# NVlabs/FoundationPose

Measured on NVIDIA H100. Metric: pose-hypotheses/sec at 640x480 RGB-D, 252 hyp, 5 refine iters, higher is better.
Workload: dtype f16

## Files before the change

foundationpose_b200/csrc/fp_attn_tc.cu:

```cuda
#include "fp_attn.cuh"
#include "fp_common.cuh"
#include "fp_gemm.cuh"
#include "fp_wgmma.cuh"

namespace fp {

int encode_map_f16(CUtensorMap* map, const void* base, int rank, const uint64_t* dims, const uint64_t* strides_bytes,
                   const uint32_t* box);
int num_sms();

namespace {

constexpr int T = 400;
constexpr int DH = 128;
constexpr int kQTiles = (T + 127) / 128;
constexpr int kKeys = 80;
constexpr int kChunks = T / kKeys;
constexpr int kKVSlab = kKeys * 128;
constexpr int kKVStage = 4 * kKVSlab;
constexpr int kKVStages = 3;
constexpr int kQSlab = 128 * 128;
constexpr int kQStage = 2 * kQSlab;
constexpr int kQStages = 2;
constexpr int kOffKV = 0;
constexpr int kOffQ = kOffKV + kKVStages * kKVStage;
constexpr int kOffBar = kOffQ + kQStages * kQStage;
constexpr int kSmem = kOffBar + 256 + 1024;
constexpr int kThreadsTc = 384;

__device__ __forceinline__ void tma_load_3d(const CUtensorMap* map, uint64_t* bar, void* dst, int c0, int c1, int c2) {
  asm volatile(
      "cp.async.bulk.tensor.3d.shared::cluster.global.mbarrier::complete_tx::bytes [%0], [%1, {%3, %4, %5}], [%2];" ::"r"(
          smem_u32(dst)),
      "l"(reinterpret_cast<uint64_t>(map)), "r"(smem_u32(bar)), "r"(c0), "r"(c1), "r"(c2)
      : "memory");
}
__device__ __forceinline__ void tma_store_4d(const CUtensorMap* map, const void* src, int c0, int c1, int c2, int c3) {
  asm volatile("cp.async.bulk.tensor.4d.global.shared::cta.bulk_group [%0, {%2, %3, %4, %5}], [%1];" ::"l"(
                   reinterpret_cast<uint64_t>(map)),
               "r"(smem_u32(src)), "r"(c0), "r"(c1), "r"(c2), "r"(c3)
               : "memory");
}

struct TcParams {
  int q_col, k_col, v_col;
  int group_col_stride;
  float scale_log2e;
  int B, H, G;
};

__global__ void __launch_bounds__(kThreadsTc, 1)
    attn_tc_kernel(const __grid_constant__ CUtensorMap map_kv,
                   const __grid_constant__ CUtensorMap map_q,
                   const __grid_constant__ CUtensorMap map_o,
                   const TcParams p) {
  extern __shared__ uint8_t smem_raw[];
  uint8_t* smem = reinterpret_cast<uint8_t*>((reinterpret_cast<uintptr_t>(smem_raw) + 1023) & ~uintptr_t(1023));
  uint64_t* bars = reinterpret_cast<uint64_t*>(smem + kOffBar);
  uint64_t* q_full = bars;
  uint64_t* q_empty = bars + kQStages;
  uint64_t* kv_full = bars + 2 * kQStages;
  uint64_t* kv_empty = bars + 2 * kQStages + kKVStages;

  const int total = p.B * p.H * p.G * kQTiles;

  if (threadIdx.x == 0) {
    tma_prefetch_desc(&map_kv);
    tma_prefetch_desc(&map_q);
    tma_prefetch_desc(&map_o);
    for (int i = 0; i < kQStages; ++i) {
      mbar_init(&q_full[i], 1);
      mbar_init(&q_empty[i], 2);
    }
    for (int i = 0; i < kKVStages; ++i) {
      mbar_init(&kv_full[i], 1);
      mbar_init(&kv_empty[i], 256);
    }
    mbar_fence_init();
  }
  __syncthreads();
  pdl_trigger();
  pdl_wait();

  auto unit = [&](int u, int& b, int& h, int& g, int& gcol, int& qt) {
    qt = u % kQTiles;
    const int w = u / kQTiles;
    b = w % p.B;
    h = (w / p.B) % p.H;
    g = w / (p.B * p.H);
    gcol = g * p.group_col_stride + h * DH;
  };

  if (threadIdx.x < 128) {
    if (threadIdx.x == 0) {
      int qs = 0, qph = 0, ks = 0, kph = 0;
      for (int u = blockIdx.x; u < total; u += gridDim.x) {
        int b, h, g, gcol, qt;
        unit(u, b, h, g, gcol, qt);
        mbar_wait(&q_empty[qs], qph ^ 1);
        mbar_expect_tx(&q_full[qs], kQStage);
        for (int s = 0; s < 2; ++s)
          tma_load_3d(&map_q, &q_full[qs], smem + kOffQ + qs * kQStage + s * kQSlab, gcol + p.q_col + s * 64, qt * 128, b);
        if (++qs == kQStages) {
          qs = 0;
          qph ^= 1;
        }
        for (int c = 0; c < kChunks; ++c) {
          mbar_wait(&kv_empty[ks], kph ^ 1);
          mbar_expect_tx(&kv_full[ks], kKVStage);
          uint8_t* st = smem + kOffKV + ks * kKVStage;
          for (int s = 0; s < 2; ++s) {
            tma_load_3d(&map_kv, &kv_full[ks], st + s * kKVSlab, gcol + p.k_col + s * 64, c * kKeys, b);
            tma_load_3d(&map_kv, &kv_full[ks], st + (2 + s) * kKVSlab, gcol + p.v_col + s * 64, c * kKeys, b);
          }
          if (++ks == kKVStages) {
            ks = 0;
            kph ^= 1;
          }
        }
      }
    }
    return;
  }

  const int ct = threadIdx.x - 128;
  const int cw = ct >> 7;
  const int lane = threadIdx.x & 31;
  const int r0 = 64 * cw + 16 * ((ct >> 5) & 3) + (lane >> 2);
  const int cq = 2 * (lane & 3);
  const bool leader = ((ct & 127) == 0);
  const float c = p.scale_log2e;
  float s_acc[kKeys / 2], o[DH / 2];
#pragma unroll
  for (int i = 0; i < kKeys / 2; ++i) s_acc[i] = 0.f;
  int qs = 0, qph = 0, ks = 0, kph = 0;
  for (int u = blockIdx.x; u < total; u += gridDim.x) {
    int b, h, g, gcol, qt;
    unit(u, b, h, g, gcol, qt);
#pragma unroll
    for (int i = 0; i < DH / 2; ++i) o[i] = 0.f;
    float m[2] = {-INFINITY, -INFINITY}, l[2] = {0.f, 0.f};
    mbar_wait(&q_full[qs], qph);
    const uint32_t qbase = smem_u32(smem + kOffQ + qs * kQStage) + (uint32_t)cw * 8192u;
    for (int ch = 0; ch < kChunks; ++ch) {
      mbar_wait(&kv_full[ks], kph);
      const uint32_t kvbase = smem_u32(smem + kOffKV + ks * kKVStage);
      wgmma_fence();
#pragma unroll
      for (int kk = 0; kk < 8; ++kk) {
        const int s = kk >> 2, k = kk & 3;
        Wgmma<kKeys>::ss(s_acc, gmma_desc_sw128(qbase + s * kQSlab) + (uint64_t)(2 * k),
                         gmma_desc_sw128(kvbase + s * kKVSlab) + (uint64_t)(2 * k), kk > 0 ? 1u : 0u);
      }
      wgmma_commit();
      wgmma_wait<0>();
      fence_regs(s_acc);
      float mx[2] = {m[0], m[1]};
#pragma unroll
      for (int j = 0; j < kKeys / 8; ++j) {
        mx[0] = fmaxf(mx[0], fmaxf(s_acc[4 * j], s_acc[4 * j + 1]));
        mx[1] = fmaxf(mx[1], fmaxf(s_acc[4 * j + 2], s_acc[4 * j + 3]));
      }
      float mc[2], alpha[2];
#pragma unroll
      for (int hh = 0; hh < 2; ++hh) {
        mx[hh] = fmaxf(mx[hh], __shfl_xor_sync(0xffffffffu, mx[hh], 1));
        mx[hh] = fmaxf(mx[hh], __shfl_xor_sync(0xffffffffu, mx[hh], 2));
        alpha[hh] = exp2f((m[hh] - mx[hh]) * c);
        m[hh] = mx[hh];
        mc[hh] = mx[hh] * c;
        l[hh] *= alpha[hh];
      }
#pragma unroll
      for (int j = 0; j < DH / 8; ++j) {
        o[4 * j] *= alpha[0];
        o[4 * j + 1] *= alpha[0];
        o[4 * j + 2] *= alpha[1];
        o[4 * j + 3] *= alpha[1];
      }
      uint32_t pa[kKeys / 16][4];
#pragma unroll
      for (int j = 0; j < kKeys / 8; ++j) {
#pragma unroll
        for (int hh = 0; hh < 2; ++hh) {
          const float p0 = exp2f(fmaf(s_acc[4 * j + 2 * hh], c, -mc[hh]));
          const float p1 = exp2f(fmaf(s_acc[4 * j + 2 * hh + 1], c, -mc[hh]));
          l[hh] += p0 + p1;
          pa[j >> 1][(j & 1) * 2 + hh] = pack_half2(p0, p1);
        }
      }
      wgmma_fence();
#pragma unroll
      for (int kk = 0; kk < kKeys / 16; ++kk)
        Wgmma<DH>::rs_mn(o, pa[kk], gmma_desc_mn_sw128(kvbase + 2 * kKVSlab + kk * 16 * 128, kKVSlab), 1u);
      wgmma_commit();
      wgmma_wait<0>();
      fence_regs(o);
      mbar_arrive(&kv_empty[ks]);
      if (++ks == kKVStages) {
        ks = 0;
        kph ^= 1;
      }
    }
    float inv[2];
#pragma unroll
    for (int hh = 0; hh < 2; ++hh) {
      l[hh] += __shfl_xor_sync(0xffffffffu, l[hh], 1);
      l[hh] += __shfl_xor_sync(0xffffffffu, l[hh], 2);
      inv[hh] = 1.f / l[hh];
    }
    uint8_t* qst = smem + kOffQ + qs * kQStage;
#pragma unroll
    for (int j = 0; j < DH / 8; ++j) {
#pragma unroll
      for (int hh = 0; hh < 2; ++hh) {
        const int row = r0 + 8 * hh;
        *reinterpret_cast<uint32_t*>(qst + (j >> 3) * kQSlab + row * 128 + ((((uint32_t)j & 7u) ^ (uint32_t)(row & 7)) << 4) +
                                     cq * 2) = pack_half2(o[4 * j + 2 * hh] * inv[hh], o[4 * j + 2 * hh + 1] * inv[hh]);
      }
    }
    asm volatile("fence.proxy.async.shared::cta;" ::: "memory");
    asm volatile("bar.sync %0, 128;" ::"r"(1 + cw) : "memory");
    if (leader) {
      for (int s = 0; s < 2; ++s)
        tma_store_4d(&map_o, qst + s * kQSlab + cw * 8192, h * DH + s * 64, qt * 128 + 64 * cw, b, g);
      asm volatile("cp.async.bulk.commit_group;" ::: "memory");
      asm volatile("cp.async.bulk.wait_group.read 0;" ::: "memory");
      mbar_arrive(&q_empty[qs]);
    }
    if (++qs == kQStages) {
      qs = 0;
      qph ^= 1;
    }
  }
  if (leader) asm volatile("cp.async.bulk.wait_group 0;" ::: "memory");
}

}

int attn_tc_launch(const AttnParams& p, cudaStream_t stream) {
  FP_REQUIRE(p.T == T && p.n_heads == 4, "wgmma attention is specialised for T=400, 4 heads of 128");
  FP_REQUIRE(p.ld_out == 512, "wgmma attention writes [*, 512] rows");
  static std::atomic<unsigned long long> attr_mask{0};
  if (!device_bit_test(attr_mask)) {
    FP_CUDA_OK(cudaFuncSetAttribute(attn_tc_kernel, cudaFuncAttributeMaxDynamicSharedMemorySize, kSmem));
    device_bit_set(attr_mask);
  }
  if (p.B == 0) return 0;
  CUtensorMap mkv, mq, mo;
  const uint64_t E = 2;
  uint64_t d3[3] = {(uint64_t)p.ld, (uint64_t)T, (uint64_t)p.B};
  uint64_t s3[2] = {(uint64_t)p.ld * E, (uint64_t)p.ld * E * T};
  uint32_t bkv[3] = {64, (uint32_t)kKeys, 1}, bq[3] = {64, 128, 1};
  int rc = encode_map_f16(&mkv, p.qkv, 3, d3, s3, bkv);
  if (rc) return rc;
  rc = encode_map_f16(&mq, p.qkv, 3, d3, s3, bq);
  if (rc) return rc;
  uint64_t d4[4] = {512, (uint64_t)T, (uint64_t)p.B, (uint64_t)p.n_groups};
  uint64_t s4[3] = {512 * E, 512 * E * T, (uint64_t)p.out_group_stride * E};
  if (p.n_groups == 1) s4[2] = 512 * E * T * p.B;
  uint32_t bo[4] = {64, 64, 1, 1};
  rc = encode_map_f16(&mo, p.out, 4, d4, s4, bo);
  if (rc) return rc;
  TcParams tp;
  tp.q_col = p.q_off;
  tp.k_col = p.k_off;
  tp.v_col = p.v_off;
  tp.group_col_stride = p.group_col_stride;
  tp.scale_log2e = p.scale * 1.4426950408889634f;
  tp.B = p.B;
  tp.H = p.n_heads;
  tp.G = p.n_groups;
  const int total = p.B * p.n_heads * p.n_groups * kQTiles;
  const int sms = num_sms();
  FP_REQUIRE(sms > 0, "no CUDA device");
  dim3 grid(total < sms ? total : sms);
  FP_CUDA_OK(launch_pdl(attn_tc_kernel, grid, dim3(kThreadsTc), kSmem, stream, 1, mkv, mq, mo, tp));
  note_launches(1);
  FP_CUDA_OK(cudaGetLastError());
  return 0;
}

}
```

Before: 3859.

## Rework wgmma attention into 64-row query blocks with split K/V rings

Adds a new default attention kernel where each consumer warpgroup handles a 64-row query block, and a scheduler packs the seven blocks of each pair of (batch, head, group) units into items, including a shared tail item. This avoids the padding waste of 128-row tiles over T=400 (four tiles covering 512 rows). K and V now flow through separate 4-stage rings, and the S=QK^T of the next chunk is issued before the softmax of the current one, so wgmma overlaps with exp work. The old kernel stays available behind an environment variable. The cost is more complex ring bookkeeping and smaller per-warpgroup tiles, which may lower tensor-core efficiency per instruction.

```diff
diff --git a/foundationpose_b200/csrc/fp_attn_tc.cu b/foundationpose_b200/csrc/fp_attn_tc.cu
--- a/foundationpose_b200/csrc/fp_attn_tc.cu
+++ b/foundationpose_b200/csrc/fp_attn_tc.cu
@@ -13,10 +13,35 @@
 
 constexpr int T = 400;
 constexpr int DH = 128;
-constexpr int kQTiles = (T + 127) / 128;
 constexpr int kKeys = 80;
 constexpr int kChunks = T / kKeys;
 constexpr int kKVSlab = kKeys * 128;
+constexpr int kThreadsTc = 384;
+
+__device__ __forceinline__ void tma_load_3d(const CUtensorMap* map, uint64_t* bar, void* dst, int c0, int c1, int c2) {
+  asm volatile(
+      "cp.async.bulk.tensor.3d.shared::cluster.global.mbarrier::complete_tx::bytes [%0], [%1, {%3, %4, %5}], [%2];" ::"r"(
+          smem_u32(dst)),
+      "l"(reinterpret_cast<uint64_t>(map)), "r"(smem_u32(bar)), "r"(c0), "r"(c1), "r"(c2)
+      : "memory");
+}
+__device__ __forceinline__ void tma_store_4d(const CUtensorMap* map, const void* src, int c0, int c1, int c2, int c3) {
+  asm volatile("cp.async.bulk.tensor.4d.global.shared::cta.bulk_group [%0, {%2, %3, %4, %5}], [%1];" ::"l"(
+                   reinterpret_cast<uint64_t>(map)),
+               "r"(smem_u32(src)), "r"(c0), "r"(c1), "r"(c2), "r"(c3)
+               : "memory");
+}
+
+struct TcParams {
+  int q_col, k_col, v_col;
+  int group_col_stride;
+  float scale_log2e;
+  int B, H, G;
+};
+
+namespace legacy {
+
+constexpr int kQTiles = (T + 127) / 128;
 constexpr int kKVStage = 4 * kKVSlab;
 constexpr int kKVStages = 3;
 constexpr int kQSlab = 128 * 128;
@@ -26,34 +51,12 @@
 constexpr int kOffQ = kOffKV + kKVStages * kKVStage;
 constexpr int kOffBar = kOffQ + kQStages * kQStage;
 constexpr int kSmem = kOffBar + 256 + 1024;
-constexpr int kThreadsTc = 384;
-
-__device__ __forceinline__ void tma_load_3d(const CUtensorMap* map, uint64_t* bar, void* dst, int c0, int c1, int c2) {
-  asm volatile(
-      "cp.async.bulk.tensor.3d.shared::cluster.global.mbarrier::complete_tx::bytes [%0], [%1, {%3, %4, %5}], [%2];" ::"r"(
-          smem_u32(dst)),
-      "l"(reinterpret_cast<uint64_t>(map)), "r"(smem_u32(bar)), "r"(c0), "r"(c1), "r"(c2)
-      : "memory");
-}
-__device__ __forceinline__ void tma_store_4d(const CUtensorMap* map, const void* src, int c0, int c1, int c2, int c3) {
-  asm volatile("cp.async.bulk.tensor.4d.global.shared::cta.bulk_group [%0, {%2, %3, %4, %5}], [%1];" ::"l"(
-                   reinterpret_cast<uint64_t>(map)),
-               "r"(smem_u32(src)), "r"(c0), "r"(c1), "r"(c2), "r"(c3)
-               : "memory");
-}
-
-struct TcParams {
-  int q_col, k_col, v_col;
-  int group_col_stride;
-  float scale_log2e;
-  int B, H, G;
-};
 
 __global__ void __launch_bounds__(kThreadsTc, 1)
-    attn_tc_kernel(const __grid_constant__ CUtensorMap map_kv,
-                   const __grid_constant__ CUtensorMap map_q,
-                   const __grid_constant__ CUtensorMap map_o,
-                   const TcParams p) {
+    attn_tc_kernel_legacy(const __grid_constant__ CUtensorMap map_kv,
+                          const __grid_constant__ CUtensorMap map_q,
+                          const __grid_constant__ CUtensorMap map_o,
+                          const TcParams p) {
   extern __shared__ uint8_t smem_raw[];
   uint8_t* smem = reinterpret_cast<uint8_t*>((reinterpret_cast<uintptr_t>(smem_raw) + 1023) & ~uintptr_t(1023));
   uint64_t* bars = reinterpret_cast<uint64_t*>(smem + kOffBar);
@@ -238,20 +241,337 @@
 
 }
 
+constexpr int kBlockRows = 64;
+constexpr int kUnitItems = 7;
+constexpr int kRingStages = 4;
+constexpr int kRingStage = 2 * kKVSlab;
+constexpr int kBlkSlab = kBlockRows * 128;
+constexpr int kBlkBuf = 2 * kBlkSlab;
+constexpr int kOffK = 0;
+constexpr int kOffV = kOffK + kRingStages * kRingStage;
+constexpr int kOffQ = kOffV + kRingStages * kRingStage;
+constexpr int kOffO = kOffQ + 2 * kBlkBuf;
+constexpr int kOffBar = kOffO + 2 * kBlkBuf;
+constexpr int kSmem = kOffBar + 256 + 1024;
+constexpr int kProducerRegs = 40;
+constexpr int kConsumerRegs = 232;
+
+struct TcItem {
+  int unit[2], blk[2];
+  bool two;
+};
+
+__device__ __forceinline__ TcItem tc_item(int i, int units) {
+  const int r = i % kUnitItems;
+  const int u0 = 2 * (i / kUnitItems), u1 = u0 + 1;
+  TcItem it;
+  if (r < 3 || (r < 6 && u1 < units)) {
+    const int u = r < 3 ? u0 : u1;
+    const int pr = r < 3 ? r : r - 3;
+    it.unit[0] = it.unit[1] = u;
+    it.blk[0] = 2 * pr;
+    it.blk[1] = 2 * pr + 1;
+    it.two = false;
+  } else {
+    it.unit[0] = u0;
+    it.blk[0] = it.blk[1] = 6;
+    it.unit[1] = u1 < units ? u1 : -1;
+    it.two = u1 < units;
+  }
+  return it;
+}
+
+__host__ __device__ __forceinline__ int tc_items(int units) { return kUnitItems * (units / 2) + (units & 1 ? 4 : 0); }
+
+struct Ring {
+  int stage = 0, phase = 0, pos = 0;
+
+  __device__ __forceinline__ int take(uint64_t* full) {
+    const int s = stage;
+    mbar_wait(&full[s], phase);
+    if (++stage == kRingStages) {
+      stage = 0;
+      phase ^= 1;
+    }
+    ++pos;
+    return s;
+  }
+  __device__ __forceinline__ int take_at(int at, uint64_t* full, uint64_t* empty) {
+    while (pos < at) mbar_arrive(&empty[take(full)]);
+    return take(full);
+  }
+  __device__ __forceinline__ void finish(int n, uint64_t* full, uint64_t* empty) {
+    while (pos < n) mbar_arrive(&empty[take(full)]);
+    pos = 0;
+  }
+};
+
+__global__ void __launch_bounds__(kThreadsTc, 1)
+    attn_tc_kernel(const __grid_constant__ CUtensorMap map_kv,
+                   const __grid_constant__ CUtensorMap map_q,
+                   const __grid_constant__ CUtensorMap map_o,
+                   const TcParams p) {
+  extern __shared__ uint8_t smem_raw[];
+  uint8_t* smem = reinterpret_cast<uint8_t*>((reinterpret_cast<uintptr_t>(smem_raw) + 1023) & ~uintptr_t(1023));
+  uint64_t* bars = reinterpret_cast<uint64_t*>(smem + kOffBar);
+  uint64_t* k_full = bars;
+  uint64_t* k_empty = bars + kRingStages;
+  uint64_t* v_full = bars + 2 * kRingStages;
+  uint64_t* v_empty = bars + 3 * kRingStages;
+  uint64_t* q_full = bars + 4 * kRingStages;
+  uint64_t* q_empty = q_full + 2;
+
+  const int units = p.B * p.H * p.G;
+  const int total = tc_items(units);
+
+  if (threadIdx.x == 0) {
+    tma_prefetch_desc(&map_kv);
+    tma_prefetch_desc(&map_q);
+    tma_prefetch_desc(&map_o);
+    for (int i = 0; i < kRingStages; ++i) {
+      mbar_init(&k_full[i], 1);
+      mbar_init(&k_empty[i], 256);
+      mbar_init(&v_full[i], 1);
+      mbar_init(&v_empty[i], 256);
+    }
+    for (int w = 0; w < 2; ++w) {
+      mbar_init(&q_full[w], 1);
+      mbar_init(&q_empty[w], 128);
+    }
+    mbar_fence_init();
+  }
+  __syncthreads();
+  pdl_trigger();
+  pdl_wait();
+
+  auto unit_cols = [&](int u, int& b, int& h, int& g, int& gcol) {
+    b = u % p.B;
+    h = (u / p.B) % p.H;
+    g = u / (p.B * p.H);
+    gcol = g * p.group_col_stride + h * DH;
+  };
+
+  if (threadIdx.x < 128) {
+    regs_release<kProducerRegs>();
+    if (threadIdx.x == 0) {
+      int ks = 0, kph = 0, vs = 0, vph = 0;
+      uint32_t qph[2] = {0, 0};
+      auto fill = [&](uint64_t* full, uint64_t* empty, int& st, int& ph, int off, int col, int chunk, int b) {
+        mbar_wait(&empty[st], ph ^ 1);
+        mbar_expect_tx(&full[st], kRingStage);
+        for (int s = 0; s < 2; ++s)
+          tma_load_3d(&map_kv, &full[st], smem + off + st * kRingStage + s * kKVSlab, col + s * 64, chunk * kKeys, b);
+        if (++st == kRingStages) {
+          st = 0;
+          ph ^= 1;
+        }
+      };
+      for (int i = blockIdx.x; i < total; i += gridDim.x) {
+        const TcItem it = tc_item(i, units);
+        int b[2], gcol[2];
+#pragma unroll
+        for (int w = 0; w < 2; ++w) {
+          if (it.unit[w] < 0) continue;
+          int h, g;
+          unit_cols(it.unit[w], b[w], h, g, gcol[w]);
+          mbar_wait(&q_empty[w], qph[w] ^ 1);
+          qph[w] ^= 1;
+          mbar_expect_tx(&q_full[w], kBlkBuf);
+          for (int s = 0; s < 2; ++s)
+            tma_load_3d(&map_q, &q_full[w], smem + kOffQ + w * kBlkBuf + s * kBlkSlab, gcol[w] + p.q_col + s * 64,
+                        it.blk[w] * kBlockRows, b[w]);
+        }
+        const int streams = it.two ? 2 : 1;
+        for (int c = 0; c <= kChunks; ++c) {
+          if (c < kChunks)
+#pragma unroll
+            for (int w = 0; w < 2; ++w)
+              if (w < streams) fill(k_full, k_empty, ks, kph, kOffK, gcol[w] + p.k_col, c, b[w]);
+          if (c > 0)
+#pragma unroll
+            for (int w = 0; w < 2; ++w)
+              if (w < streams) fill(v_full, v_empty, vs, vph, kOffV, gcol[w] + p.v_col, c - 1, b[w]);
+        }
+      }
+    }
+    return;
+  }
+
+  regs_acquire<kConsumerRegs>();
+  const int ct = threadIdx.x - 128;
+  const int cw = ct >> 7;
+  const int lane = threadIdx.x & 31;
+  const int r0 = 16 * ((ct >> 5) & 3) + (lane >> 2);
+  const int cq = 2 * (lane & 3);
+  const bool leader = ((ct & 127) == 0);
+  const float c = p.scale_log2e;
+  const uint32_t qbase = smem_u32(smem + kOffQ + cw * kBlkBuf);
+  uint8_t* ost = smem + kOffO + cw * kBlkBuf;
+  float s_acc[2][kKeys / 2], o[DH / 2];
+  uint32_t pa[kKeys / 16][4];
+  Ring kr, vr;
+  uint32_t qph = 0;
+
+  auto issue_s = [&](float (&acc)[kKeys / 2], int kst) {
+    const uint32_t kbase = smem_u32(smem + kOffK + kst * kRingStage);
+    wgmma_fence();
+#pragma unroll
+    for (int kk = 0; kk < 8; ++kk) {
+      const int s = kk >> 2, k = kk & 3;
+      Wgmma<kKeys>::ss(acc, gmma_desc_sw128(qbase + s * kBlkSlab) + (uint64_t)(2 * k),
+                       gmma_desc_sw128(kbase + s * kKVSlab) + (uint64_t)(2 * k), kk > 0 ? 1u : 0u);
+    }
+    wgmma_commit();
+  };
+
+  for (int i = blockIdx.x; i < total; i += gridDim.x) {
+    const TcItem it = tc_item(i, units);
+    const int fills = it.two ? 2 * kChunks : kChunks;
+    const int my_unit = cw ? it.unit[1] : it.unit[0], my_blk = cw ? it.blk[1] : it.blk[0];
+    if (my_unit < 0) {
+      kr.finish(fills, k_full, k_empty);
+      vr.finish(fills, v_full, v_empty);
+      continue;
+    }
+    const int at0 = it.two ? cw : 0, at_step = it.two ? 2 : 1;
+    int b, h, g, gcol;
+    unit_cols(my_unit, b, h, g, gcol);
+#pragma unroll
+    for (int e = 0; e < DH / 2; ++e) o[e] = 0.f;
+    float m[2] = {-INFINITY, -INFINITY}, l[2] = {0.f, 0.f};
+    int k_cur, k_next = 0, v_prev = 0;
+    mbar_wait(&q_full[cw], qph);
+    qph ^= 1;
+    k_cur = kr.take_at(at0, k_full, k_empty);
+    issue_s(s_acc[0], k_cur);
+#pragma unroll
+    for (int ch = 0; ch < kChunks; ++ch) {
+      float(&sc)[kKeys / 2] = s_acc[ch & 1];
+      if (ch + 1 < kChunks) {
+        k_next = kr.take_at(at0 + (ch + 1) * at_step, k_full, k_empty);
+        issue_s(s_acc[(ch + 1) & 1], k_next);
+      }
+      if (ch > 0 && ch + 1 < kChunks)
+        wgmma_wait<2>();
+      else
+        wgmma_wait<1>();
+      fence_regs(sc);
+      mbar_arrive(&k_empty[k_cur]);
+      k_cur = k_next;
+      if (ch + 1 == kChunks) mbar_arrive(&q_empty[cw]);
+      float mx[2] = {m[0], m[1]};
+#pragma unroll
+      for (int j = 0; j < kKeys / 8; ++j) {
+        mx[0] = fmaxf(mx[0], fmaxf(sc[4 * j], sc[4 * j + 1]));
+        mx[1] = fmaxf(mx[1], fmaxf(sc[4 * j + 2], sc[4 * j + 3]));
+      }
+      float mc[2], alpha[2];
+#pragma unroll
+      for (int hh = 0; hh < 2; ++hh) {
+        mx[hh] = fmaxf(mx[hh], __shfl_xor_sync(0xffffffffu, mx[hh], 1));
+        mx[hh] = fmaxf(mx[hh], __shfl_xor_sync(0xffffffffu, mx[hh], 2));
+        alpha[hh] = exp2f((m[hh] - mx[hh]) * c);
+        m[hh] = mx[hh];
+        mc[hh] = mx[hh] * c;
+        l[hh] *= alpha[hh];
+      }
+#pragma unroll
+      for (int j = 0; j < kKeys / 8; ++j) {
+#pragma unroll
+        for (int hh = 0; hh < 2; ++hh) {
+          const float p0 = exp2f(fmaf(sc[4 * j + 2 * hh], c, -mc[hh]));
+          const float p1 = exp2f(fmaf(sc[4 * j + 2 * hh + 1], c, -mc[hh]));
+          l[hh] += p0 + p1;
+          sc[4 * j + 2 * hh] = p0;
+          sc[4 * j + 2 * hh + 1] = p1;
+        }
+      }
+      fence_regs(sc);
+      if (ch > 0) {
+        if (ch + 1 < kChunks)
+          wgmma_wait<1>();
+        else
+          wgmma_wait<0>();
+        fence_regs(o);
+      }
+#pragma unroll
+      for (int j = 0; j < DH / 8; ++j) {
+        o[4 * j] *= alpha[0];
+        o[4 * j + 1] *= alpha[0];
+        o[4 * j + 2] *= alpha[1];
+        o[4 * j + 3] *= alpha[1];
+      }
+#pragma unroll
+      for (int j = 0; j < kKeys / 8; ++j)
+#pragma unroll
+        for (int hh = 0; hh < 2; ++hh) pa[j >> 1][(j & 1) * 2 + hh] = pack_half2(sc[4 * j + 2 * hh], sc[4 * j + 2 * hh + 1]);
+      if (ch > 0) mbar_arrive(&v_empty[v_prev]);
+      v_prev = vr.take_at(at0 + ch * at_step, v_full, v_empty);
+      const uint32_t vbase = smem_u32(smem + kOffV + v_prev * kRingStage);
+      wgmma_fence();
+#pragma unroll
+      for (int kk = 0; kk < kKeys / 16; ++kk)
+        Wgmma<DH>::rs_mn(o, pa[kk], gmma_desc_mn_sw128(vbase + kk * 16 * 128, kKVSlab), 1u);
+      wgmma_commit();
+    }
+    wgmma_wait<0>();
+    fence_regs(o);
+    mbar_arrive(&v_empty[v_prev]);
+    kr.finish(fills, k_full, k_empty);
+    vr.finish(fills, v_full, v_empty);
+    float inv[2];
+#pragma unroll
+    for (int hh = 0; hh < 2; ++hh) {
+      l[hh] += __shfl_xor_sync(0xffffffffu, l[hh], 1);
+      l[hh] += __shfl_xor_sync(0xffffffffu, l[hh], 2);
+      inv[hh] = 1.f / l[hh];
+    }
+    if (leader) asm volatile("cp.async.bulk.wait_group.read 0;" ::: "memory");
+    asm volatile("bar.sync %0, 128;" ::"r"(1 + cw) : "memory");
+#pragma unroll
+    for (int j = 0; j < DH / 8; ++j) {
+#pragma unroll
+      for (int hh = 0; hh < 2; ++hh) {
+        const int row = r0 + 8 * hh;
+        *reinterpret_cast<uint32_t*>(ost + (j >> 3) * kBlkSlab + row * 128 +
+                                     ((((uint32_t)j & 7u) ^ (uint32_t)(row & 7)) << 4) + cq * 2) =
+            pack_half2(o[4 * j + 2 * hh] * inv[hh], o[4 * j + 2 * hh + 1] * inv[hh]);
+      }
+    }
+    asm volatile("fence.proxy.async.shared::cta;" ::: "memory");
+    asm volatile("bar.sync %0, 128;" ::"r"(1 + cw) : "memory");
+    if (leader) {
+      for (int s = 0; s < 2; ++s) tma_store_4d(&map_o, ost + s * kBlkSlab, h * DH + s * 64, my_blk * kBlockRows, b, g);
+      asm volatile("cp.async.bulk.commit_group;" ::: "memory");
+    }
+  }
+  if (leader) asm volatile("cp.async.bulk.wait_group 0;" ::: "memory");
+}
+
+}
+
+static bool attn_legacy() {
+  const char* e = getenv("FPOSE_ATTN_LEGACY");
+  return e && e[0] == '1';
+}
+
 int attn_tc_launch(const AttnParams& p, cudaStream_t stream) {
   FP_REQUIRE(p.T == T && p.n_heads == 4, "wgmma attention is specialised for T=400, 4 heads of 128");
   FP_REQUIRE(p.ld_out == 512, "wgmma attention writes [*, 512] rows");
   static std::atomic<unsigned long long> attr_mask{0};
   if (!device_bit_test(attr_mask)) {
+    FP_CUDA_OK(cudaFuncSetAttribute(legacy::attn_tc_kernel_legacy, cudaFuncAttributeMaxDynamicSharedMemorySize,
+                                    legacy::kSmem));
     FP_CUDA_OK(cudaFuncSetAttribute(attn_tc_kernel, cudaFuncAttributeMaxDynamicSharedMemorySize, kSmem));
     device_bit_set(attr_mask);
   }
   if (p.B == 0) return 0;
+  const bool leg = attn_legacy();
   CUtensorMap mkv, mq, mo;
   const uint64_t E = 2;
   uint64_t d3[3] = {(uint64_t)p.ld, (uint64_t)T, (uint64_t)p.B};
   uint64_t s3[2] = {(uint64_t)p.ld * E, (uint64_t)p.ld * E * T};
-  uint32_t bkv[3] = {64, (uint32_t)kKeys, 1}, bq[3] = {64, 128, 1};
+  uint32_t bkv[3] = {64, (uint32_t)kKeys, 1}, bq[3] = {64, leg ? 128u : (uint32_t)kBlockRows, 1};
   int rc = encode_map_f16(&mkv, p.qkv, 3, d3, s3, bkv);
   if (rc) return rc;
   rc = encode_map_f16(&mq, p.qkv, 3, d3, s3, bq);
@@ -271,11 +591,16 @@
   tp.B = p.B;
   tp.H = p.n_heads;
   tp.G = p.n_groups;
-  const int total = p.B * p.n_heads * p.n_groups * kQTiles;
+  const int units = p.B * p.n_heads * p.n_groups;
+  const int total = leg ? units * legacy::kQTiles : tc_items(units);
   const int sms = num_sms();
   FP_REQUIRE(sms > 0, "no CUDA device");
   dim3 grid(total < sms ? total : sms);
-  FP_CUDA_OK(launch_pdl(attn_tc_kernel, grid, dim3(kThreadsTc), kSmem, stream, 1, mkv, mq, mo, tp));
+  if (leg)
+    FP_CUDA_OK(launch_pdl(legacy::attn_tc_kernel_legacy, grid, dim3(kThreadsTc), legacy::kSmem, stream, 1, mkv, mq, mo,
+                          tp));
+  else
+    FP_CUDA_OK(launch_pdl(attn_tc_kernel, grid, dim3(kThreadsTc), kSmem, stream, 1, mkv, mq, mo, tp));
   note_launches(1);
   FP_CUDA_OK(cudaGetLastError());
   return 0;
```

Result: no change. 3864 (median of 6 runs) (+0.1%).
